# cv-core/MIT-Driverless-CV-TrainingInfra

Hardware: AMD Instinct MI355X
Metric: images/sec training (YOLOv3 416^2 + RektNet 80^2) (higher is better)
Workload: dtype bf16; 1 GPU; CVC-YOLOv3 yolo_baseline 416x416 classes=80, train step (fwd+bwd+Adam), 32 img/GPU; global_batch=32, parallelism=dp1, hipgraph=False, optimizer=FusedAdam

## Files before the change

mit-driverless-cv-traininginfra_amd/csrc/pw_bwd.hip:

```cpp
#include "common.h"
#include "bn_fuse.h"

struct PwbArgs {
  const void* dy; const void* x; const void* wd; void* dx; const void* addsrc; float* ws;
  int ldy, ldx, lddx, ldadd;
  int M, Cin, Cout;
  int slab_px, nslabs, slices;
  BnFuseArgs fuse;
};

namespace {

constexpr int NT = 512, NW = 8;
constexpr int BP = 32;
constexpr int NS = 64;
constexpr int T64 = 2 * 2048 + 128;
constexpr int SPITCH = 136;
typedef __attribute__((address_space(3))) void lds_void_t;
typedef __attribute__((ext_vector_type(4))) short s16x4_t;
typedef __attribute__((ext_vector_type(8))) short s16x8_t;


__device__ __forceinline__ int swz(int row) { return (row >> 1) & 2; }
__device__ __forceinline__ unsigned lds_u32(const unsigned char* p) {
  return (unsigned)(size_t)(const __attribute__((address_space(3))) unsigned char*)p;
}
__device__ __forceinline__ uint2 lds_rd64(unsigned addr) {
  uint2 v;
  asm volatile("ds_read_b64 %0, %1" : "=v"(v) : "v"(addr) : "memory");
  return v;
}
template <int OFF> __device__ __forceinline__ s16x4_t lds_tr16(unsigned addr) {
  s16x4_t v;
  asm volatile("ds_read_b64_tr_b16 %0, %1 offset:%2" : "=v"(v) : "v"(addr), "n"(OFF) : "memory");
  return v;
}

template <int CO4, int S, bool ADD, bool FUSE>
__global__ __launch_bounds__(NT) void pw_bwd_kernel(PwbArgs a) {
  constexpr int KB = 2 * CO4;
  constexpr int NX = 1 + (ADD ? 1 : 0) + (FUSE ? 1 : 0);
  constexpr int WD_BYTES = KB * 4096;
  constexpr int STG = KB * 2048 + NX * T64;
  constexpr int STAGING = WD_BYTES + S * STG;
  constexpr int DUMP = STAGING + BP * SPITCH;
  constexpr int NCHUNK = 2 * KB + 4 * NX;
  constexpr int NPW = (NCHUNK + NW - 1) / NW;
  extern __shared__ __attribute__((aligned(1024))) unsigned char smem[];

  const int xcd = (int)(blockIdx.x & 7), seq = (int)(blockIdx.x >> 3);
  const int slab = xcd + 8 * (seq / a.slices), slice = seq % a.slices;
  if (slab >= a.nslabs) return;
  const int tid = threadIdx.x, lane = tid & 63;
  const int wave = __builtin_amdgcn_readfirstlane(tid >> 6);
  const int px0 = slab * a.slab_px;
  const int px_end = min(a.M, px0 + a.slab_px);
  const int ntiles = (px_end - px0 + BP - 1) / BP;
  const int ci0 = slice * NS;

  const __amdgpu_buffer_rsrc_t rwd = __builtin_amdgcn_make_buffer_rsrc(const_cast<void*>(a.wd), 0, (unsigned)a.Cin * (unsigned)a.Cout * 2u, 0x00020000);

  const int lrow = lane >> 2, lslot = (lane & 3) ^ swz(lrow);
#define PWB_SETUP(I)                                                                                                               \
  const int c##I = wave + NW * I;                                                                                 \
  const int cc##I = c##I - 2 * KB, t##I = cc##I >> 2, b##I = (cc##I >> 1) & 1, g##I = c##I & 1;                                      \
  const bool isdy##I = c##I < 2 * KB, live##I = c##I < NCHUNK;                                                                       \
  const int k##I = isdy##I ? 0 : (t##I == 0 ? 1 : ((ADD && t##I == 1) ? 2 : 3));                      \
  const void* bp##I = k##I == 0 ? a.dy : (k##I == 1 ? a.x : (k##I == 2 ? a.addsrc : a.fuse.y));                                     \
  const unsigned ld##I = (unsigned)(k##I == 0 ? a.ldy : (k##I == 1 ? a.ldx : (k##I == 2 ? a.ldadd : a.fuse.ldy)));                  \
  const unsigned pitch##I = live##I ? ld##I * 2u : 0u;                                                                              \
  const __amdgpu_buffer_rsrc_t rs##I = __builtin_amdgcn_make_buffer_rsrc(const_cast<void*>(live##I ? bp##I : a.dy), 0,              \
                                                                         live##I ? (unsigned)px_end * ld##I * 2u : 0u, 0x00020000); \
  const int ch##I = isdy##I ? (c##I >> 1) * 32 : ci0 + b##I * 32;                                                                   \
  const unsigned voff##I = live##I ? (unsigned)(g##I * 16 + lrow) * pitch##I + (unsigned)(ch##I + lslot * 8) * 2u : 0u;             \
  const unsigned ldso##I = !live##I ? (unsigned)(DUMP - WD_BYTES)                                                                   \
                                    : (isdy##I ? (unsigned)((c##I >> 1) * 2048 + g##I * 1024)                                       \
                                               : (unsigned)(KB * 2048 + t##I * T64 + b##I * (2048 + 128) + g##I * 1024));           \
  const unsigned smul##I = live##I ? (unsigned)STG : 0u;
  PWB_SETUP(0) PWB_SETUP(1) PWB_SETUP(2) PWB_SETUP(3) PWB_SETUP(4) PWB_SETUP(5)
#undef PWB_SETUP
  static_assert(NPW <= 6, "six DMA roles per wave");
#define PWB_ISSUE_ONE(I, PROW_, SLOT_)                                                                                             \
  if constexpr (I < NPW)                                                                                                          \
    __builtin_amdgcn_raw_ptr_buffer_load_lds(rs##I, (lds_void_t*)(smem + WD_BYTES + (unsigned)(SLOT_) * smul##I + ldso##I), 16,      \
                                             (int)voff##I, (int)((PROW_) * pitch##I), 0, 0)
#define PWB_ISSUE_TILE(T_, SLOT_)                                                                                                  \
  do {                                                                                                                           \
    const unsigned prow__ = (unsigned)(px0 + (T_) * BP);                                                                         \
    PWB_ISSUE_ONE(0, prow__, SLOT_); PWB_ISSUE_ONE(1, prow__, SLOT_); PWB_ISSUE_ONE(2, prow__, SLOT_);                           \
    PWB_ISSUE_ONE(3, prow__, SLOT_); PWB_ISSUE_ONE(4, prow__, SLOT_); PWB_ISSUE_ONE(5, prow__, SLOT_);                           \
  } while (0)

#pragma unroll
  for (int i = 0; i < (4 * KB) / NW; ++i) {
    const int c = wave + NW * i, kb = c >> 2, g = c & 3;
    const unsigned vo = (unsigned)(ci0 + g * 16 + lrow) * (unsigned)a.Cout * 2u + (unsigned)(kb * 32 + lslot * 8) * 2u;
    __builtin_amdgcn_raw_ptr_buffer_load_lds(rwd, (lds_void_t*)(smem + kb * 4096 + g * 1024), 16, (int)vo, 0, 0, 0);
  }
  int issued = 0;
  for (; issued < S - 1 && issued < ntiles; ++issued) PWB_ISSUE_TILE(issued, issued);

  const int r16 = lane & 15, q4 = lane >> 4;
  const int offF = r16 * 64 + ((q4 ^ swz(r16)) << 4);
  const int cb = wave & 3, pb = wave >> 2;
  const unsigned char* const pWd = smem + (cb * 16) * 64 + offF;
  const int trow = q4 * 4 + (r16 >> 2);
  const int tsub = (r16 & 1) * 8, tq = (r16 & 3) >> 1;
  const int wc = wave >> 1, wn = wave & 1;
  const int erow = tid >> 4, ecg = tid & 15;
  const int eblk = ecg >> 3, eslot = (ecg & 7) >> 1, esub = (ecg & 1) * 8;
  const int eoff64 = eblk * (2048 + 128) + erow * 64 + ((eslot ^ swz(erow & 15)) << 4) + esub;
  bf16_t* __restrict__ dxp = reinterpret_cast<bf16_t*>(a.dx);
  const unsigned stg_wr = lds_u32(smem) + (unsigned)(STAGING + (pb * 16 + r16) * SPITCH + cb * 32 + q4 * 8);

  float fs[4], fb[4], fm[4], sg[4], sx[4];
  if constexpr (FUSE) {
#pragma unroll
    for (int e = 0; e < 4; ++e) {
      const int n = ci0 + ecg * 4 + e;
      fs[e] = a.fuse.scale[n]; fb[e] = a.fuse.shift[n]; fm[e] = a.fuse.mean[n]; sg[e] = 0.f; sx[e] = 0.f;
    }
  }

  f32x4_t accw[CO4][2];
#pragma unroll
  for (int i = 0; i < CO4; ++i)
#pragma unroll
    for (int j = 0; j < 2; ++j) accw[i][j] = f32x4_t{0.f, 0.f, 0.f, 0.f};

  int slot = 0, islot = issued % S;
  for (int t = 0; t < ntiles; ++t) {
    const int newer = issued - 1 - t;
    if (S > 2 && newer >= S - 2) asm volatile("s_waitcnt vmcnt(%0)" ::"n"((S > 2 ? S - 2 : 0) * NPW) : "memory");
    else asm volatile("s_waitcnt vmcnt(0)" ::: "memory");
    asm volatile("s_waitcnt lgkmcnt(0)" ::: "memory");
    __builtin_amdgcn_s_barrier();
    if (issued < ntiles) {
      PWB_ISSUE_TILE(issued, islot);
      ++issued;
      islot = islot + 1 == S ? 0 : islot + 1;
    }
    const unsigned char* stg = smem + WD_BYTES + slot * STG;

    {
      f32x4_t acc = f32x4_t{0.f, 0.f, 0.f, 0.f};
      const unsigned char* pB = stg + (pb * 16) * 64 + offF;
#pragma unroll
      for (int kb = 0; kb < KB; ++kb) {
        const bf16x8_t fa = *reinterpret_cast<const bf16x8_t*>(pWd + kb * 4096);
        const bf16x8_t fbv = *reinterpret_cast<const bf16x8_t*>(pB + kb * 2048);
        acc = __builtin_amdgcn_mfma_f32_16x16x32_bf16(fa, fbv, acc, 0, 0, 0);
      }
      uint2 pk;
      pk.x = pack_bf16x2(acc[0], acc[1]); pk.y = pack_bf16x2(acc[2], acc[3]);
      asm volatile("ds_write_b64 %0, %1" ::"v"(stg_wr), "v"(pk) : "memory");
    }

    {
      bf16x8_t fx[2], fd[CO4];
      const unsigned xb = lds_u32(stg) + (unsigned)(KB * 2048 + wn * (2048 + 128) + trow * 64 + tsub);
#pragma unroll
      for (int j = 0; j < 2; ++j) {
        const unsigned ad = xb + (unsigned)((((2 * j + tq) ^ swz(trow)) << 4));
        const s16x4_t lo = lds_tr16<0>(ad), hi = lds_tr16<1024>(ad);
        const s16x8_t v = {lo[0], lo[1], lo[2], lo[3], hi[0], hi[1], hi[2], hi[3]};
        fx[j] = __builtin_bit_cast(bf16x8_t, v);
      }
      const unsigned db = lds_u32(stg) + (unsigned)(trow * 64 + tsub);
#pragma unroll
      for (int i = 0; i < CO4; ++i) {
        const int gblk = wc * CO4 + i;
        const unsigned ad = db + (unsigned)((gblk >> 1) * 2048) + (unsigned)((((2 * (gblk & 1) + tq) ^ swz(trow)) << 4));
        const s16x4_t lo = lds_tr16<0>(ad), hi = lds_tr16<1024>(ad);
        const s16x8_t v = {lo[0], lo[1], lo[2], lo[3], hi[0], hi[1], hi[2], hi[3]};
        fd[i] = __builtin_bit_cast(bf16x8_t, v);
      }
      asm volatile("s_waitcnt lgkmcnt(0)" ::: "memory");
#pragma unroll
      for (int j = 0; j < 2; ++j) asm volatile("" : "+v"(fx[j]));
#pragma unroll
      for (int i = 0; i < CO4; ++i) asm volatile("" : "+v"(fd[i]));
#pragma unroll
      for (int i = 0; i < CO4; ++i)
#pragma unroll
        for (int j = 0; j < 2; ++j) accw[i][j] = __builtin_amdgcn_mfma_f32_16x16x32_bf16(fd[i], fx[j], accw[i][j], 0, 0, 0);
    }

    asm volatile("s_waitcnt lgkmcnt(0)" ::: "memory");
    __builtin_amdgcn_s_barrier();
    {
      const int p = px0 + t * BP + erow;
      const unsigned sbase = lds_u32(stg) + (unsigned)(KB * 2048 + eoff64);
      uint2 d = lds_rd64(lds_u32(smem) + (unsigned)(STAGING + erow * SPITCH + ecg * 8)), q = d, yq = d;
      if constexpr (ADD) q = lds_rd64(sbase + T64);
      if constexpr (FUSE) yq = lds_rd64(sbase + (NX - 1) * T64);
      asm volatile("s_waitcnt lgkmcnt(0)" : "+v"(d), "+v"(q), "+v"(yq)::"memory");
      float v[4];
      v[0] = __uint_as_float(d.x << 16); v[1] = __uint_as_float(d.x & 0xffff0000u);
      v[2] = __uint_as_float(d.y << 16); v[3] = __uint_as_float(d.y & 0xffff0000u);
      if constexpr (ADD) {
        v[0] += __uint_as_float(q.x << 16); v[1] += __uint_as_float(q.x & 0xffff0000u);
        v[2] += __uint_as_float(q.y << 16); v[3] += __uint_as_float(q.y & 0xffff0000u);
        d.x = pack_bf16x2(v[0], v[1]); d.y = pack_bf16x2(v[2], v[3]);
      }
      if (p < px_end) *reinterpret_cast<uint2*>(dxp + (size_t)p * a.lddx + ci0 + ecg * 4) = d;
      if constexpr (FUSE) {
        if (p < px_end) {
          float yv[4];
          yv[0] = __uint_as_float(yq.x << 16); yv[1] = __uint_as_float(yq.x & 0xffff0000u);
          yv[2] = __uint_as_float(yq.y << 16); yv[3] = __uint_as_float(yq.y & 0xffff0000u);
          v[0] = __uint_as_float(d.x << 16); v[1] = __uint_as_float(d.x & 0xffff0000u);
          v[2] = __uint_as_float(d.y << 16); v[3] = __uint_as_float(d.y & 0xffff0000u);
#pragma unroll
          for (int e = 0; e < 4; ++e) {
            const float pre = __builtin_fmaf(yv[e], fs[e], fb[e]);
            const float g = (a.fuse.act != 0 && !(pre > 0.f)) ? v[e] * a.fuse.slope : v[e];
            sg[e] += g;
            sx[e] += g * (yv[e] - fm[e]);
          }
        }
      }
    }
    slot = slot + 1 == S ? 0 : slot + 1;
  }

  {
    float* __restrict__ wsp = a.ws + (size_t)slab * a.Cout * a.Cin + ci0 + wn * 32 + r16;
#pragma unroll
    for (int i = 0; i < CO4; ++i)
#pragma unroll
      for (int j = 0; j < 2; ++j)
#pragma unroll
        for (int rr = 0; rr < 4; ++rr) {
          const int co = (wc * CO4 + i) * 16 + q4 * 4 + rr;
          wsp[(size_t)co * a.Cin + j * 16] = accw[i][j][rr];
        }
  }
  if constexpr (FUSE) {
#pragma unroll
    for (int e = 0; e < 4; ++e) {
      sg[e] += __shfl_xor(sg[e], 16, 64); sx[e] += __shfl_xor(sx[e], 16, 64);
      sg[e] += __shfl_xor(sg[e], 32, 64); sx[e] += __shfl_xor(sx[e], 32, 64);
    }
    asm volatile("s_waitcnt vmcnt(0) lgkmcnt(0)" ::: "memory");
    __builtin_amdgcn_s_barrier();
    float* red = reinterpret_cast<float*>(smem + WD_BYTES);
    if (lane < 16) {
#pragma unroll
      for (int e = 0; e < 4; ++e) { red[(wave * 2 + 0) * 64 + lane * 4 + e] = sg[e]; red[(wave * 2 + 1) * 64 + lane * 4 + e] = sx[e]; }
    }
    __syncthreads();
    if (tid < 128) {
      float tot = 0.f;
#pragma unroll
      for (int w = 0; w < NW; ++w) tot += red[w * 128 + tid];
      const int which = tid >> 6, c = tid & 63;
      a.fuse.partial[(size_t)(a.fuse.row_base + slab) * 2 * a.Cin + (size_t)which * a.Cin + ci0 + c] = tot;
    }
  }
}

#undef PWB_ISSUE_TILE
#undef PWB_ISSUE_ONE

template <int CO4, int S, bool ADD, bool FUSE>
int launch_pwb(const PwbArgs& a, hipStream_t st) {
  constexpr int KB = 2 * CO4, NX = 1 + (ADD ? 1 : 0) + (FUSE ? 1 : 0);
  constexpr int LDS = KB * 4096 + S * (KB * 2048 + NX * T64) + BP * SPITCH + 1024;
  static_assert(LDS <= 160 * 1024, "LDS budget");
  auto kern = pw_bwd_kernel<CO4, S, ADD, FUSE>;
  static DynLds dyn_lds;
  if (hipError_t e = mdcv_dyn_lds(dyn_lds, reinterpret_cast<const void*>(kern), LDS); e != hipSuccess) return (int)e;
  const unsigned grid = (unsigned)(8 * cdiv(a.nslabs, 8) * a.slices);
  MDCV_LAUNCH(kern, dim3(grid), dim3(NT), LDS, st, a);
  MDCV_CHECK_LAUNCH();
  return MDCV_OK;
}

template <int CO4, int S>
int launch_pwb2(const PwbArgs& a, hipStream_t st) {
  const bool add = a.addsrc != nullptr, fuse = a.fuse.y != nullptr;
  if (add) return fuse ? launch_pwb<CO4, S, true, true>(a, st) : launch_pwb<CO4, S, true, false>(a, st);
  return fuse ? launch_pwb<CO4, S, false, true>(a, st) : launch_pwb<CO4, S, false, false>(a, st);
}

int device_cus() {
  static int cus[64] = {};
  int dev = 0;
  if (hipGetDevice(&dev) != hipSuccess || dev < 0 || dev >= 64) return 256;
  if (!cus[dev]) {
    int n = 0;
    cus[dev] = (hipDeviceGetAttribute(&n, hipDeviceAttributeMultiprocessorCount, dev) == hipSuccess && n >= 8) ? n : 256;
  }
  return cus[dev];
}

int pwb_lds_bytes(int Cout) {
  const int KB = Cout / 32, S = Cout >= 512 ? 2 : 3;
  return KB * 4096 + S * (KB * 2048 + 3 * T64) + BP * SPITCH + 1024;
}

}

extern "C" {

int mdcv_pw_bwd_slabs(int dtype, long long M, int Cin, int Cout, int ldy, int ldx, int lddx, int ldadd, int ldfy) {
  if (dtype != MDCV_BF16 || M < 1) return 0;
  if (Cout != 64 && Cout != 128 && Cout != 256 && Cout != 512) return 0;
  if (Cin < 64 || (Cin & 63)) return 0;
  if ((ldy & 7) || (ldx & 7) || (lddx & 3) || (ldadd & 7) || (ldfy & 7)) return 0;
  const long long ldmax = (long long)(ldy > ldx ? ldy : ldx) > (ldadd > ldfy ? ldadd : ldfy) ? (ldy > ldx ? ldy : ldx) : (ldadd > ldfy ? ldadd : ldfy);
  if ((M + 64) * ldmax * 2 >= (1LL << 31) || (long long)Cin * Cout * 2 >= (1LL << 31)) return 0;
  const int ncu = device_cus();
  const int per_cu = (160 * 1024) / pwb_lds_bytes(Cout);
  const int slices = Cin / NS;
  const int xcd_slots = (ncu / 8) * (per_cu < 1 ? 1 : per_cu);
  int P = 8 * (xcd_slots / slices > 0 ? xcd_slots / slices : 1);
  long long spx = ((M + P - 1) / P + BP - 1) / BP * BP;
  if (spx < 4 * BP) spx = 4 * BP;
  return (int)((M + spx - 1) / spx);
}

int mdcv_pw_bwd(int dtype, const void* dy, int ldy, const void* x, int ldx, const void* wd_packed, void* dx, int lddx, const void* addsrc,
                int ldadd, float* ws, int slabs, const void* fy, int ldfy, const float* fscale, const float* fshift, const float* fmean, int fact,
                float fslope, float* fpartial, long long M, int Cin, int Cout, void* stream) {
  if (!dy || !x || !wd_packed || !dx || !ws) return MDCV_EARG;
  if (slabs < 1 || slabs != mdcv_pw_bwd_slabs(dtype, M, Cin, Cout, ldy, ldx, lddx, addsrc ? ldadd : 8, fy ? ldfy : 8)) return MDCV_EARG;
  PwbArgs a{};
  a.dy = dy; a.x = x; a.wd = wd_packed; a.dx = dx; a.addsrc = addsrc; a.ws = ws;
  a.ldy = ldy; a.ldx = ldx; a.lddx = lddx; a.ldadd = ldadd;
  a.M = (int)M; a.Cin = Cin; a.Cout = Cout;
  a.nslabs = slabs; a.slices = Cin / NS;
  a.slab_px = (int)(((M + slabs - 1) / slabs + BP - 1) / BP * BP);
  a.fuse = BnFuseArgs{};
  if (fy) {
    if (!fscale || !fshift || !fmean || !fpartial) return MDCV_EARG;
    a.fuse.y = fy; a.fuse.ldy = ldfy; a.fuse.scale = fscale; a.fuse.shift = fshift; a.fuse.mean = fmean; a.fuse.partial = fpartial;
    a.fuse.act = fact; a.fuse.slope = fact == 2 ? 0.f : fslope; a.fuse.row_base = 0;
  }
  hipStream_t st = (hipStream_t)stream;
  switch (Cout) {
    case 64: return launch_pwb2<1, 3>(a, st);
    case 128: return launch_pwb2<2, 3>(a, st);
    case 256: return launch_pwb2<4, 3>(a, st);
    case 512: return launch_pwb2<8, 2>(a, st);
  }
  return MDCV_EARG;
}

}
```

mit-driverless-cv-traininginfra_amd/csrc/tune.h:

```cpp
#pragma once

struct MdcvTune {
  int conv_no_ut = 0;
  int conv_tall_narrow = 256;
  int conv_deep_narrow = 1;
  int conv_deep_small = 8;
  int conv_fuse_narrow = 1;
  int conv_variant = -1;
  int conv_tall_s2 = 1;
  int conv_deep_s2 = 1;
  int conv_s2_allcls = 1;
  int conv_s2_split = 512;
  int conv_s2_split_on = 1;
  int wgrad_slots = 512;
  int wgrad_bna_stages = 2;
  int wgrad_variant = 0;
  int shift_ring = 4;
  int shift_wmax_narrow = 104;
  int shift_wmax_n32 = 0;
  int shift_dil2 = 1;
  int shift_n64 = 2;
  int shift_wmax = 80;
  int shift_loop = 2;
  int shift_2d = 1;
  int shift_big = 0;
  int shift_n64_wide = 1;
  int shift_plan = 0;
  int shift_s2 = 1;
  int pw_bmp = 0;
  int pw_wres = 1;
  int stream_blocks = 0;
  int stream_tiled = 1;
  int stream_light_maxpos = 600000;
  int stream_table = 1;
  int stream_direct = 1;
  int stream_s2 = 1;
  int stream_s2_blocks = 256;
  int stream_s2_depth = 2;
  int stream_s2_lds = 160 * 1024;
  int stream_light_depth = 1;
  int stream_light_blocks = 256;
  int stream_tiled_blocks = 128;
};

extern thread_local const MdcvTune* mdcv_t_tune;
inline const MdcvTune& TUNE() { return *mdcv_t_tune; }

enum { MDCV_TUNE_CONV = 0, MDCV_TUNE_WGRAD = 1, MDCV_TUNE_PW = 2 };

inline void mdcv_tune_shift(MdcvTune& t, int ring) {
  if (ring == 63 || ring == 64) { t.shift_n64_wide = ring - 63; return; }
  if (ring == 29 || ring == 60) { t.shift_s2 = ring == 60; return; }
  if (ring == 27 || ring == 28) { t.shift_2d = ring - 27; return; }
  if (ring >= 200 && ring < 300) { t.shift_big = ring == 201 ? 384 : 0; return; }
  if (ring >= 30 && ring <= 59) { t.shift_loop = ring - 30; return; }
  if (ring == 25 || ring == 26) { t.shift_wmax_n32 = ring == 25 ? 208 : 0; return; }
  if (ring == 23 || ring == 24) { t.shift_wmax_narrow = ring == 23 ? 104 : 0; return; }
  if (ring >= 20 && ring <= 22) { t.shift_dil2 = ring == 20 ? 2 : (ring == 21 ? 0 : 1); return; }
  if (ring >= 17 && ring <= 19) { t.shift_n64 = ring == 17 ? 1 : (ring == 18 ? 0 : 2); return; }
  if (ring >= 14 && ring <= 16) { t.shift_wmax = ring == 14 ? 80 : (ring == 15 ? 62 : 104); return; }
  if (ring >= 7) t.shift_plan = ring - 7;
  else if (ring >= 3 && ring <= 5) t.shift_ring = ring;
}
inline void mdcv_tune_apply_conv(MdcvTune& t, int v) {
  if (v == 0) return;
  if (v <= -3 && v >= -299) { mdcv_tune_shift(t, -v); return; }
  if (v == 93 || v == 92) { t.conv_fuse_narrow = v == 93; return; }
  if (v >= 60 && v < 92) { t.conv_deep_small = v - 60; return; }
  if (v >= 30 && v < 60) { t.conv_deep_narrow = v - 30; return; }
  if (v == 20 || v == 21) { t.conv_deep_s2 = v - 20; return; }
  if (v == 16 || v == 17) { t.conv_s2_allcls = v - 16; return; }
  if (v == 14 || v == 15) { t.conv_s2_split_on = v - 14; return; }
  if (v >= 4000 && v < 6000) { t.conv_s2_split = v - 4000; return; }
  if (v == 18 || v == 19) { t.conv_tall_s2 = v - 18; return; }
  if (v >= 2000 && v < 3000) { t.conv_tall_narrow = v - 2000; return; }
  if (v >= 100) { t.conv_no_ut = 1; v -= 100; }
  if (v >= 1 && v <= 12) t.conv_variant = v - 1;
}
inline void mdcv_tune_apply_wgrad(MdcvTune& t, int v) {
  if (v == 0) return;
  if (v >= 20000 && v < 30000) { t.wgrad_slots = v - 20000; return; }
  if (v >= 35000 && v < 36000) { t.stream_s2_blocks = v - 35000; return; }
  if (v >= 30000 && v < 40000) {
    const int b = v - 30000;
    if (b >= 4001 && b <= 4002) { t.stream_light_depth = b - 4000; return; }
    if (b >= 4012 && b <= 4014) { t.wgrad_bna_stages = b - 4010; return; }
    if (b == 4020 || b == 4021) { t.stream_table = b - 4020; return; }
    if (b == 4050 || b == 4051) { t.stream_direct = b - 4050; return; }
    if (b == 4060 || b == 4061) { t.stream_s2 = b - 4060; return; }
    if (b >= 4071 && b <= 4073) { t.stream_s2_depth = b - 4070; return; }
    if (b >= 4100 && b <= 4260) { t.stream_s2_lds = (b - 4100) * 1024; return; }
    if (b == 2) t.stream_light_maxpos = 600000;
    else if (b == 3) t.stream_light_maxpos = 1 << 30;
    else if (b == 5) t.stream_light_maxpos = 0;
    else if (b >= 3000 && b < 4000) t.stream_light_blocks = b - 3000;
    else t.stream_tiled_blocks = b > 0 ? b : 128;
    return;
  }
  if (v >= 1000) { const int d = (v - 1000) / 100; t.stream_tiled = !(d & 8); t.stream_blocks = ((v - 1000) % 100) * 64; return; }
  t.wgrad_variant = v;
}
inline void mdcv_tune_apply_pw(MdcvTune& t, int v) {
  if (v == 1000 || v == 1001) { t.pw_wres = v - 1000; return; }
  if (v == 64 || v == 32 || v == 16) t.pw_bmp = v;
}

struct TuneScope {
  MdcvTune t;
  const MdcvTune* prev;
  int dtype;
  TuneScope(int dtype_arg, int family) : prev(mdcv_t_tune), dtype(dtype_arg & 0xff) {
    const int code = dtype_arg >> 8;
    if (code != 0) {
      if (family == MDCV_TUNE_CONV) mdcv_tune_apply_conv(t, code);
      else if (family == MDCV_TUNE_WGRAD) mdcv_tune_apply_wgrad(t, code);
      else mdcv_tune_apply_pw(t, code);
      mdcv_t_tune = &t;
    }
  }
  explicit TuneScope(const MdcvTune& forced) : t(forced), prev(mdcv_t_tune), dtype(0) { mdcv_t_tune = &t; }
  ~TuneScope() { mdcv_t_tune = prev; }
  TuneScope(const TuneScope&) = delete;
  TuneScope& operator=(const TuneScope&) = delete;
};
#define MDCV_TUNE_ENTRY(dtype_var, family) const TuneScope tune_scope__((dtype_var), (family)); (dtype_var) = tune_scope__.dtype
```

mit-driverless-cv-traininginfra_amd/engine.py:

```python
import os

import torch

from . import _lib
from ._lib import F32, BF16, ACT_NONE, ACT_LEAKY, ACT_RELU, tuned


_POISON = os.environ.get("MDCV_POISON", "0") == "1"
_REDZONE = int(os.environ.get("MDCV_REDZONE", "0"))
_RZ_BYTE = 0xA5


def _alloc(n, dtype, device, zero, plan):
    if not _REDZONE:
        t = (torch.zeros if zero else torch.empty)(n, dtype=dtype, device=device)
        if not zero and _POISON and t.is_floating_point():
            t.fill_(float("nan"))
        return t
    es = torch.empty(0, dtype=dtype).element_size()
    raw = torch.full((n * es + _REDZONE,), _RZ_BYTE, dtype=torch.uint8, device=device)
    t = raw[:n * es].view(dtype)
    if zero:
        t.zero_()
    plan.__dict__.setdefault("redzones", []).append((raw, n * es))
# ... 261 lines not shown
        self.call(lst, self.L.bn_act_fwd, self.dtype, a.ptr, a.ldc, None, None, None, 0, None, None, b.ptr if b is not None else None,
                  b.ldc if b is not None else 0, out.ptr, out.ldc, out.M, out.C, ACT_NONE, 0.0)

    def _alloc_like(self, a):
        return self.new_act(a.B, a.H, a.W, a.C)

    def emit_input(self, B, C, H, W):
        a = self.new_act(B, H, W, C)
        node = TNode(a, needs_grad=False, name="input")
        holder = {"src": None}
        L, dt = self.L, self.dtype

        def convert(stream):
            x = holder["src"]
            return L.nchw_to_nhwc(dt, x.data_ptr(), a.ptr, B, C, H, W, a.ldc, a.C, stream)
        convert.__name__ = "nchw_to_nhwc"
        self.fwd.append((convert, ()))
        return node, holder

    def emit_pack(self, cs, need_dgrad):
        if need_dgrad and cs.wd is None:
            cs.wd = _alloc(cs.cin_pad * cs.kh * cs.kw * cs.cout_pad, self.tdtype, self.device, True, self)
        self.pack_list.append(cs)
        self.layer_marks.append(len(self.fwd))

    def stats_rows(self, cs, x, y):
        return int(self.L.conv2d_stats_rows_geom(self.cdt, x.B, y.H, y.W, cs.cin_pad, cs.cout_pad, cs.kh, cs.kw, cs.stride, cs.pad,
                                                 cs.dil, x.ldc))

    def emit_conv_fwd(self, cs, x, y, stats_partial=None):
        assert x.C == cs.cin_pad and y.C == cs.cout_pad, (x.C, cs.cin_pad, y.C, cs.cout_pad)
        self.call(self.fwd, self.L.conv2d, self.cdt, 0, x.ptr, x.ldc, cs.wf.data_ptr(), y.ptr, y.ldc,
                  cs.bias_pad.data_ptr() if cs.bias_pad is not None else None, None, 0,
                  stats_partial.data_ptr() if stats_partial is not None else None,
                  x.B, x.H, x.W, cs.cin_pad, y.H, y.W, cs.cout_pad, cs.kh, cs.kw, cs.stride, cs.pad, cs.dil)

    def emit_conv_bwd(self, cs, xnode, y_shape_act, dy, x_wgrad=None):
        L, dt = self.L, self.dtype
        x = xnode.act
        if x_wgrad is None and self._emit_pw_bwd1(cs, xnode, dy):
            return
        xw = x_wgrad if x_wgrad is not None else x
        cin_w = xw.C if x_wgrad is not None else cs.cin_pad
        if self.wgrad_after_dgrad and cs.kh == 3 and cs.stride == 1:
            self._emit_dgrad(cs, xnode, dy)
            self._emit_wgrad_single(cs, xw, dy, cin_w)
        else:
            self._emit_wgrad_single(cs, xw, dy, cin_w)
            self._emit_dgrad(cs, xnode, dy)

    wgrad_after_dgrad = False

    pw_bwd1 = True

    def _emit_pw_bwd1(self, cs, xnode, dy):
        L, dt = self.L, self.dtype
        x = xnode.act
        if not self.pw_bwd1 or dt != BF16 or not xnode.needs_grad or cs.wd is None:
            return False
        if (cs.kh, cs.kw, cs.stride, cs.pad) != (1, 1, 1, 0) or x.C != cs.cin_pad or dy.C != cs.cout_pad:
            return False
        slabs = int(L.pw_bwd_slabs(dt, x.M, cs.cin_pad, cs.cout_pad, dy.ldc, x.ldc, 8, 8, 8))
        if slabs < 1:
            return False
        out, add = self.grad_target(xnode)
        assert slabs == int(L.pw_bwd_slabs(dt, x.M, cs.cin_pad, cs.cout_pad, dy.ldc, x.ldc, out.ldc, add.ldc if add is not None else 8, 8))
        gw = self.param_grad(cs.weight)
        ws = self.f32(slabs * cs.cout_pad * cs.cin_pad, zero=False)
        args = [dt, dy.ptr, dy.ldc, x.ptr, x.ldc, cs.wd.data_ptr(), out.ptr, out.ldc, add.ptr if add is not None else None,
                add.ldc if add is not None else 0, ws.data_ptr(), slabs, None, 0, None, None, None, 0, 0.0, None, x.M, cs.cin_pad, cs.cout_pad]
        self.dgrad_entries[out.ptr] = dict(
            idx=len(self.bwd), out=out, used=False, pwb=args,
            geom=(x.B, dy.H, dy.W, cs.cout_pad, x.H, x.W, cs.cin_pad, cs.kh, cs.kw, cs.stride, cs.pad, cs.dil), head=(dy.ptr, dy.ldc))
        self.call(self.bwd, L.pw_bwd, *args)

        def wreduce(stream, ws=ws, gw=gw, slabs=slabs, cs=cs):
            return L.wgrad_reduce(ws.data_ptr(), slabs, gw.data_ptr(), 0, cs.cout_pad, cs.cout, cs.cin_pad, cs.cin, 1, stream)
        wreduce.__name__ = "conv2d_wgrad"
        wreduce.info = (x.B, x.H, x.W, cs.cin_pad, dy.H, dy.W, cs.cout_pad, 0, 1, slabs)
        self.bwd.append((wreduce, ()))
        self.pw_bwd1_count = getattr(self, "pw_bwd1_count", 0) + 1
        return True

    def _emit_wgrad_single(self, cs, xw, dy, cin_w):
        L, dt = self.L, self.dtype
        gw = self.param_grad(cs.weight)
        splits = int(L.conv2d_wgrad_splits_geom(self.wdt, xw.B, xw.H, xw.W, cin_w, dy.H, dy.W, cs.cout_pad, cs.kh, cs.kw, cs.stride, cs.pad,
                                                cs.dil, dy.ldc, xw.ldc))
        self.ws_floats = max(self.ws_floats, splits * cs.cout_pad * cs.kh * cs.kw * cin_w)
        plan = self

        def wgrad(stream, cs=cs, x=xw, dy=dy, gw=gw, splits=splits, cin_w=cin_w):
            return L.conv2d_wgrad(plan.wdt, dy.ptr, dy.ldc, x.ptr, x.ldc, plan.wgrad_ws(stream).data_ptr(), splits, gw.data_ptr(), 0,
                                  x.B, x.H, x.W, cin_w, cs.cin, dy.H, dy.W, cs.cout_pad, cs.cout, cs.kh, cs.kw,
                                  cs.stride, cs.pad, cs.dil, stream)
        wgrad.__name__ = "conv2d_wgrad"
        wgrad.info = (xw.B, xw.H, xw.W, cin_w, dy.H, dy.W, cs.cout_pad, cs.kh, cs.stride, splits)
        self.bwd.append((wgrad, ()))

    def _emit_dgrad(self, cs, xnode, dy):
        L, dt = self.L, self.dtype
        x = xnode.act
        if xnode.needs_grad:
            out, add = self.grad_target(xnode)
            self.dgrad_entries[out.ptr] = dict(
                idx=len(self.bwd), out=out, used=False,
                geom=(x.B, dy.H, dy.W, cs.cout_pad, x.H, x.W, cs.cin_pad, cs.kh, cs.kw, cs.stride, cs.pad, cs.dil),
                head=(dy.ptr, dy.ldc, cs.wd.data_ptr(), out.ptr, out.ldc, add.ptr if add is not None else None,
                      add.ldc if add is not None else 0))
            self.call(self.bwd, L.conv2d, self.cdt, 1, dy.ptr, dy.ldc, cs.wd.data_ptr(), out.ptr, out.ldc, None,
                      add.ptr if add is not None else None, add.ldc if add is not None else 0, None,
                      x.B, dy.H, dy.W, cs.cout_pad, x.H, x.W, cs.cin_pad, cs.kh, cs.kw, cs.stride, cs.pad, cs.dil)

    def emit_bias_grad(self, cs, dy, zero_only=False):
        gb = self.param_grad(cs.bias)
        if zero_only:
            gb.zero_()
            return
        tmp = self.f32(cs.cout_pad)
        pws = self.f32(int(self.L.colsum_ws_floats(self.dtype, dy.M, cs.cout_pad)), zero=False)
        self.call(self.bwd, self.L.colsum_f32, self.dtype, dy.ptr, dy.ldc, dy.M, cs.cout_pad, pws.data_ptr(), tmp.data_ptr())

# ... 415 lines not shown
```

Measured before the change: 2494 images/sec.

## Add 128-channel-wide Cin slices to fused pointwise backward kernel

```diff
diff --git a/mit-driverless-cv-traininginfra_amd/csrc/pw_bwd.hip b/mit-driverless-cv-traininginfra_amd/csrc/pw_bwd.hip
--- a/mit-driverless-cv-traininginfra_amd/csrc/pw_bwd.hip
+++ b/mit-driverless-cv-traininginfra_amd/csrc/pw_bwd.hip
@@ -36,16 +36,22 @@
   return v;
 }
 
-template <int CO4, int S, bool ADD, bool FUSE>
+constexpr int pwb_lds(int KB, int S, int H, int NX) { return H * KB * 4096 + S * (KB * 2048 + NX * H * T64) + H * BP * SPITCH + 1024; }
+
+template <int CO4, int S, int NS2, bool ADD, bool FUSE>
 __global__ __launch_bounds__(NT) void pw_bwd_kernel(PwbArgs a) {
+  static_assert(NS2 == 64 || NS2 == 128, "one or two 64-channel halves");
+  constexpr int H = NS2 / NS;
   constexpr int KB = 2 * CO4;
   constexpr int NX = 1 + (ADD ? 1 : 0) + (FUSE ? 1 : 0);
-  constexpr int WD_BYTES = KB * 4096;
-  constexpr int STG = KB * 2048 + NX * T64;
+  constexpr int WD_HALF = KB * 4096;
+  constexpr int WD_BYTES = H * WD_HALF;
+  constexpr int STG = KB * 2048 + NX * H * T64;
   constexpr int STAGING = WD_BYTES + S * STG;
-  constexpr int DUMP = STAGING + BP * SPITCH;
-  constexpr int NCHUNK = 2 * KB + 4 * NX;
+  constexpr int DUMP = STAGING + H * BP * SPITCH;
+  constexpr int NCHUNK = 2 * KB + 4 * NX * H;
   constexpr int NPW = (NCHUNK + NW - 1) / NW;
+  static_assert(DUMP + 1024 == pwb_lds(KB, S, H, NX), "launch_pwb sizes the same layout");
   extern __shared__ __attribute__((aligned(1024))) unsigned char smem[];
 
   const int xcd = (int)(blockIdx.x & 7), seq = (int)(blockIdx.x >> 3);
@@ -56,14 +62,15 @@
   const int px0 = slab * a.slab_px;
   const int px_end = min(a.M, px0 + a.slab_px);
   const int ntiles = (px_end - px0 + BP - 1) / BP;
-  const int ci0 = slice * NS;
+  const int ci0 = slice * NS2;
 
   const __amdgpu_buffer_rsrc_t rwd = __builtin_amdgcn_make_buffer_rsrc(const_cast<void*>(a.wd), 0, (unsigned)a.Cin * (unsigned)a.Cout * 2u, 0x00020000);
 
   const int lrow = lane >> 2, lslot = (lane & 3) ^ swz(lrow);
 #define PWB_SETUP(I)                                                                                                               \
   const int c##I = wave + NW * I;                                                                                 \
-  const int cc##I = c##I - 2 * KB, t##I = cc##I >> 2, b##I = (cc##I >> 1) & 1, g##I = c##I & 1;                                      \
+  const int cc##I = c##I - 2 * KB, im##I = cc##I >> 2, b##I = (cc##I >> 1) & 1, g##I = c##I & 1;                                     \
+  const int t##I = im##I / H, hh##I = im##I % H;                                                    \
   const bool isdy##I = c##I < 2 * KB, live##I = c##I < NCHUNK;                                                                       \
   const int k##I = isdy##I ? 0 : (t##I == 0 ? 1 : ((ADD && t##I == 1) ? 2 : 3));                      \
   const void* bp##I = k##I == 0 ? a.dy : (k##I == 1 ? a.x : (k##I == 2 ? a.addsrc : a.fuse.y));                                     \
@@ -71,11 +78,11 @@
   const unsigned pitch##I = live##I ? ld##I * 2u : 0u;                                                                              \
   const __amdgpu_buffer_rsrc_t rs##I = __builtin_amdgcn_make_buffer_rsrc(const_cast<void*>(live##I ? bp##I : a.dy), 0,              \
                                                                          live##I ? (unsigned)px_end * ld##I * 2u : 0u, 0x00020000); \
-  const int ch##I = isdy##I ? (c##I >> 1) * 32 : ci0 + b##I * 32;                                                                   \
+  const int ch##I = isdy##I ? (c##I >> 1) * 32 : ci0 + hh##I * NS + b##I * 32;                                                      \
   const unsigned voff##I = live##I ? (unsigned)(g##I * 16 + lrow) * pitch##I + (unsigned)(ch##I + lslot * 8) * 2u : 0u;             \
   const unsigned ldso##I = !live##I ? (unsigned)(DUMP - WD_BYTES)                                                                   \
                                     : (isdy##I ? (unsigned)((c##I >> 1) * 2048 + g##I * 1024)                                       \
-                                               : (unsigned)(KB * 2048 + t##I * T64 + b##I * (2048 + 128) + g##I * 1024));           \
+                                               : (unsigned)(KB * 2048 + im##I * T64 + b##I * (2048 + 128) + g##I * 1024));          \
   const unsigned smul##I = live##I ? (unsigned)STG : 0u;
   PWB_SETUP(0) PWB_SETUP(1) PWB_SETUP(2) PWB_SETUP(3) PWB_SETUP(4) PWB_SETUP(5)
 #undef PWB_SETUP
@@ -92,10 +99,10 @@
   } while (0)
 
 #pragma unroll
-  for (int i = 0; i < (4 * KB) / NW; ++i) {
-    const int c = wave + NW * i, kb = c >> 2, g = c & 3;
-    const unsigned vo = (unsigned)(ci0 + g * 16 + lrow) * (unsigned)a.Cout * 2u + (unsigned)(kb * 32 + lslot * 8) * 2u;
-    __builtin_amdgcn_raw_ptr_buffer_load_lds(rwd, (lds_void_t*)(smem + kb * 4096 + g * 1024), 16, (int)vo, 0, 0, 0);
+  for (int i = 0; i < (H * 4 * KB) / NW; ++i) {
+    const int c = wave + NW * i, hw = c / (4 * KB), kb = (c % (4 * KB)) >> 2, g = c & 3;
+    const unsigned vo = (unsigned)(ci0 + hw * NS + g * 16 + lrow) * (unsigned)a.Cout * 2u + (unsigned)(kb * 32 + lslot * 8) * 2u;
+    __builtin_amdgcn_raw_ptr_buffer_load_lds(rwd, (lds_void_t*)(smem + hw * WD_HALF + kb * 4096 + g * 1024), 16, (int)vo, 0, 0, 0);
   }
   int issued = 0;
   for (; issued < S - 1 && issued < ntiles; ++issued) PWB_ISSUE_TILE(issued, issued);
@@ -112,21 +119,26 @@
   const int eoff64 = eblk * (2048 + 128) + erow * 64 + ((eslot ^ swz(erow & 15)) << 4) + esub;
   bf16_t* __restrict__ dxp = reinterpret_cast<bf16_t*>(a.dx);
   const unsigned stg_wr = lds_u32(smem) + (unsigned)(STAGING + (pb * 16 + r16) * SPITCH + cb * 32 + q4 * 8);
-
-  float fs[4], fb[4], fm[4], sg[4], sx[4];
+  const unsigned stg_rd = lds_u32(smem) + (unsigned)(STAGING + erow * SPITCH + ecg * 8);
+
+  float fs[H][4], fb[H][4], fm[H][4], sg[H][4], sx[H][4];
   if constexpr (FUSE) {
 #pragma unroll
-    for (int e = 0; e < 4; ++e) {
-      const int n = ci0 + ecg * 4 + e;
-      fs[e] = a.fuse.scale[n]; fb[e] = a.fuse.shift[n]; fm[e] = a.fuse.mean[n]; sg[e] = 0.f; sx[e] = 0.f;
-    }
-  }
-
-  f32x4_t accw[CO4][2];
-#pragma unroll
-  for (int i = 0; i < CO4; ++i)
-#pragma unroll
-    for (int j = 0; j < 2; ++j) accw[i][j] = f32x4_t{0.f, 0.f, 0.f, 0.f};
+    for (int h = 0; h < H; ++h)
+#pragma unroll
+      for (int e = 0; e < 4; ++e) {
+        const int n = ci0 + h * NS + ecg * 4 + e;
+        fs[h][e] = a.fuse.scale[n]; fb[h][e] = a.fuse.shift[n]; fm[h][e] = a.fuse.mean[n]; sg[h][e] = 0.f; sx[h][e] = 0.f;
+      }
+  }
+
+  f32x4_t accw[H][CO4][2];
+#pragma unroll
+  for (int h = 0; h < H; ++h)
+#pragma unroll
+    for (int i = 0; i < CO4; ++i)
+#pragma unroll
+      for (int j = 0; j < 2; ++j) accw[h][i][j] = f32x4_t{0.f, 0.f, 0.f, 0.f};
 
   int slot = 0, islot = issued % S;
   for (int t = 0; t < ntiles; ++t) {
@@ -143,28 +155,39 @@
     const unsigned char* stg = smem + WD_BYTES + slot * STG;
 
     {
-      f32x4_t acc = f32x4_t{0.f, 0.f, 0.f, 0.f};
+      f32x4_t acc[H];
+#pragma unroll
+      for (int h = 0; h < H; ++h) acc[h] = f32x4_t{0.f, 0.f, 0.f, 0.f};
       const unsigned char* pB = stg + (pb * 16) * 64 + offF;
 #pragma unroll
       for (int kb = 0; kb < KB; ++kb) {
-        const bf16x8_t fa = *reinterpret_cast<const bf16x8_t*>(pWd + kb * 4096);
         const bf16x8_t fbv = *reinterpret_cast<const bf16x8_t*>(pB + kb * 2048);
-        acc = __builtin_amdgcn_mfma_f32_16x16x32_bf16(fa, fbv, acc, 0, 0, 0);
-      }
-      uint2 pk;
-      pk.x = pack_bf16x2(acc[0], acc[1]); pk.y = pack_bf16x2(acc[2], acc[3]);
-      asm volatile("ds_write_b64 %0, %1" ::"v"(stg_wr), "v"(pk) : "memory");
+#pragma unroll
+        for (int h = 0; h < H; ++h) {
+          const bf16x8_t fa = *reinterpret_cast<const bf16x8_t*>(pWd + h * WD_HALF + kb * 4096);
+          acc[h] = __builtin_amdgcn_mfma_f32_16x16x32_bf16(fa, fbv, acc[h], 0, 0, 0);
+        }
+      }
+#pragma unroll
+      for (int h = 0; h < H; ++h) {
+        uint2 pk;
+        pk.x = pack_bf16x2(acc[h][0], acc[h][1]); pk.y = pack_bf16x2(acc[h][2], acc[h][3]);
+        asm volatile("ds_write_b64 %0, %1" ::"v"(stg_wr + (unsigned)(h * BP * SPITCH)), "v"(pk) : "memory");
+      }
     }
 
     {
-      bf16x8_t fx[2], fd[CO4];
-      const unsigned xb = lds_u32(stg) + (unsigned)(KB * 2048 + wn * (2048 + 128) + trow * 64 + tsub);
-#pragma unroll
-      for (int j = 0; j < 2; ++j) {
-        const unsigned ad = xb + (unsigned)((((2 * j + tq) ^ swz(trow)) << 4));
-        const s16x4_t lo = lds_tr16<0>(ad), hi = lds_tr16<1024>(ad);
-        const s16x8_t v = {lo[0], lo[1], lo[2], lo[3], hi[0], hi[1], hi[2], hi[3]};
-        fx[j] = __builtin_bit_cast(bf16x8_t, v);
+      bf16x8_t fx[H][2], fd[CO4];
+#pragma unroll
+      for (int h = 0; h < H; ++h) {
+        const unsigned xb = lds_u32(stg) + (unsigned)(KB * 2048 + h * T64 + wn * (2048 + 128) + trow * 64 + tsub);
+#pragma unroll
+        for (int j = 0; j < 2; ++j) {
+          const unsigned ad = xb + (unsigned)((((2 * j + tq) ^ swz(trow)) << 4));
+          const s16x4_t lo = lds_tr16<0>(ad), hi = lds_tr16<1024>(ad);
+          const s16x8_t v = {lo[0], lo[1], lo[2], lo[3], hi[0], hi[1], hi[2], hi[3]};
+          fx[h][j] = __builtin_bit_cast(bf16x8_t, v);
+        }
       }
       const unsigned db = lds_u32(stg) + (unsigned)(trow * 64 + tsub);
 #pragma unroll
@@ -177,13 +200,17 @@
       }
       asm volatile("s_waitcnt lgkmcnt(0)" ::: "memory");
 #pragma unroll
-      for (int j = 0; j < 2; ++j) asm volatile("" : "+v"(fx[j]));
+      for (int h = 0; h < H; ++h)
+#pragma unroll
+        for (int j = 0; j < 2; ++j) asm volatile("" : "+v"(fx[h][j]));
 #pragma unroll
       for (int i = 0; i < CO4; ++i) asm volatile("" : "+v"(fd[i]));
 #pragma unroll
-      for (int i = 0; i < CO4; ++i)
-#pragma unroll
-        for (int j = 0; j < 2; ++j) accw[i][j] = __builtin_amdgcn_mfma_f32_16x16x32_bf16(fd[i], fx[j], accw[i][j], 0, 0, 0);
+      for (int h = 0; h < H; ++h)
+#pragma unroll
+        for (int i = 0; i < CO4; ++i)
+#pragma unroll
+          for (int j = 0; j < 2; ++j) accw[h][i][j] = __builtin_amdgcn_mfma_f32_16x16x32_bf16(fd[i], fx[h][j], accw[h][i][j], 0, 0, 0);
     }
 
     asm volatile("s_waitcnt lgkmcnt(0)" ::: "memory");
@@ -191,32 +218,41 @@
     {
       const int p = px0 + t * BP + erow;
       const unsigned sbase = lds_u32(stg) + (unsigned)(KB * 2048 + eoff64);
-      uint2 d = lds_rd64(lds_u32(smem) + (unsigned)(STAGING + erow * SPITCH + ecg * 8)), q = d, yq = d;
-      if constexpr (ADD) q = lds_rd64(sbase + T64);
-      if constexpr (FUSE) yq = lds_rd64(sbase + (NX - 1) * T64);
-      asm volatile("s_waitcnt lgkmcnt(0)" : "+v"(d), "+v"(q), "+v"(yq)::"memory");
-      float v[4];
-      v[0] = __uint_as_float(d.x << 16); v[1] = __uint_as_float(d.x & 0xffff0000u);
-      v[2] = __uint_as_float(d.y << 16); v[3] = __uint_as_float(d.y & 0xffff0000u);
-      if constexpr (ADD) {
-        v[0] += __uint_as_float(q.x << 16); v[1] += __uint_as_float(q.x & 0xffff0000u);
-        v[2] += __uint_as_float(q.y << 16); v[3] += __uint_as_float(q.y & 0xffff0000u);
-        d.x = pack_bf16x2(v[0], v[1]); d.y = pack_bf16x2(v[2], v[3]);
-      }
-      if (p < px_end) *reinterpret_cast<uint2*>(dxp + (size_t)p * a.lddx + ci0 + ecg * 4) = d;
-      if constexpr (FUSE) {
-        if (p < px_end) {
-          float yv[4];
-          yv[0] = __uint_as_float(yq.x << 16); yv[1] = __uint_as_float(yq.x & 0xffff0000u);
-          yv[2] = __uint_as_float(yq.y << 16); yv[3] = __uint_as_float(yq.y & 0xffff0000u);
-          v[0] = __uint_as_float(d.x << 16); v[1] = __uint_as_float(d.x & 0xffff0000u);
-          v[2] = __uint_as_float(d.y << 16); v[3] = __uint_as_float(d.y & 0xffff0000u);
-#pragma unroll
-          for (int e = 0; e < 4; ++e) {
-            const float pre = __builtin_fmaf(yv[e], fs[e], fb[e]);
-            const float g = (a.fuse.act != 0 && !(pre > 0.f)) ? v[e] * a.fuse.slope : v[e];
-            sg[e] += g;
-            sx[e] += g * (yv[e] - fm[e]);
+      uint2 d[H], q[H], yq[H];
+#pragma unroll
+      for (int h = 0; h < H; ++h) {
+        d[h] = lds_rd64(stg_rd + (unsigned)(h * BP * SPITCH)); q[h] = d[h]; yq[h] = d[h];
+        if constexpr (ADD) q[h] = lds_rd64(sbase + (unsigned)((H + h) * T64));
+        if constexpr (FUSE) yq[h] = lds_rd64(sbase + (unsigned)(((NX - 1) * H + h) * T64));
+      }
+      asm volatile("s_waitcnt lgkmcnt(0)" ::: "memory");
+#pragma unroll
+      for (int h = 0; h < H; ++h) asm volatile("" : "+v"(d[h]), "+v"(q[h]), "+v"(yq[h]));
+#pragma unroll
+      for (int h = 0; h < H; ++h) {
+        float v[4];
+        v[0] = __uint_as_float(d[h].x << 16); v[1] = __uint_as_float(d[h].x & 0xffff0000u);
+        v[2] = __uint_as_float(d[h].y << 16); v[3] = __uint_as_float(d[h].y & 0xffff0000u);
+        if constexpr (ADD) {
+          v[0] += __uint_as_float(q[h].x << 16); v[1] += __uint_as_float(q[h].x & 0xffff0000u);
+          v[2] += __uint_as_float(q[h].y << 16); v[3] += __uint_as_float(q[h].y & 0xffff0000u);
+          d[h].x = pack_bf16x2(v[0], v[1]); d[h].y = pack_bf16x2(v[2], v[3]);
+        }
+        if (p < px_end) *reinterpret_cast<uint2*>(dxp + (size_t)p * a.lddx + ci0 + h * NS + ecg * 4) = d[h];
+        if constexpr (FUSE) {
+          if (p < px_end) {
+            float yv[4];
+            yv[0] = __uint_as_float(yq[h].x << 16); yv[1] = __uint_as_float(yq[h].x & 0xffff0000u);
+            yv[2] = __uint_as_float(yq[h].y << 16); yv[3] = __uint_as_float(yq[h].y & 0xffff0000u);
+            v[0] = __uint_as_float(d[h].x << 16); v[1] = __uint_as_float(d[h].x & 0xffff0000u);
+            v[2] = __uint_as_float(d[h].y << 16); v[3] = __uint_as_float(d[h].y & 0xffff0000u);
+#pragma unroll
+            for (int e = 0; e < 4; ++e) {
+              const float pre = __builtin_fmaf(yv[e], fs[h][e], fb[h][e]);
+              const float g = (a.fuse.act != 0 && !(pre > 0.f)) ? v[e] * a.fuse.slope : v[e];
+              sg[h][e] += g;
+              sx[h][e] += g * (yv[e] - fm[h][e]);
+            }
           }
         }
       }
@@ -225,36 +261,46 @@
   }
 
   {
-    float* __restrict__ wsp = a.ws + (size_t)slab * a.Cout * a.Cin + ci0 + wn * 32 + r16;
-#pragma unroll
-    for (int i = 0; i < CO4; ++i)
-#pragma unroll
-      for (int j = 0; j < 2; ++j)
-#pragma unroll
-        for (int rr = 0; rr < 4; ++rr) {
-          const int co = (wc * CO4 + i) * 16 + q4 * 4 + rr;
-          wsp[(size_t)co * a.Cin + j * 16] = accw[i][j][rr];
-        }
+#pragma unroll
+    for (int h = 0; h < H; ++h) {
+      float* __restrict__ wsp = a.ws + (size_t)slab * a.Cout * a.Cin + ci0 + h * NS + wn * 32 + r16;
+#pragma unroll
+      for (int i = 0; i < CO4; ++i)
+#pragma unroll
+        for (int j = 0; j < 2; ++j)
+#pragma unroll
+          for (int rr = 0; rr < 4; ++rr) {
+            const int co = (wc * CO4 + i) * 16 + q4 * 4 + rr;
+            wsp[(size_t)co * a.Cin + j * 16] = accw[h][i][j][rr];
+          }
+    }
   }
   if constexpr (FUSE) {
 #pragma unroll
-    for (int e = 0; e < 4; ++e) {
-      sg[e] += __shfl_xor(sg[e], 16, 64); sx[e] += __shfl_xor(sx[e], 16, 64);
-      sg[e] += __shfl_xor(sg[e], 32, 64); sx[e] += __shfl_xor(sx[e], 32, 64);
-    }
+    for (int h = 0; h < H; ++h)
+#pragma unroll
+      for (int e = 0; e < 4; ++e) {
+        sg[h][e] += __shfl_xor(sg[h][e], 16, 64); sx[h][e] += __shfl_xor(sx[h][e], 16, 64);
+        sg[h][e] += __shfl_xor(sg[h][e], 32, 64); sx[h][e] += __shfl_xor(sx[h][e], 32, 64);
+      }
     asm volatile("s_waitcnt vmcnt(0) lgkmcnt(0)" ::: "memory");
     __builtin_amdgcn_s_barrier();
     float* red = reinterpret_cast<float*>(smem + WD_BYTES);
+    static_assert(NW * 2 * NS2 * 4 <= S * STG, "the wave sums fit the ring");
     if (lane < 16) {
 #pragma unroll
-      for (int e = 0; e < 4; ++e) { red[(wave * 2 + 0) * 64 + lane * 4 + e] = sg[e]; red[(wave * 2 + 1) * 64 + lane * 4 + e] = sx[e]; }
+      for (int h = 0; h < H; ++h)
+#pragma unroll
+        for (int e = 0; e < 4; ++e) {
+          red[(wave * 2 + 0) * NS2 + h * NS + lane * 4 + e] = sg[h][e]; red[(wave * 2 + 1) * NS2 + h * NS + lane * 4 + e] = sx[h][e];
+        }
     }
     __syncthreads();
-    if (tid < 128) {
+    if (tid < 2 * NS2) {
       float tot = 0.f;
 #pragma unroll
-      for (int w = 0; w < NW; ++w) tot += red[w * 128 + tid];
-      const int which = tid >> 6, c = tid & 63;
+      for (int w = 0; w < NW; ++w) tot += red[w * 2 * NS2 + tid];
+      const int which = tid / NS2, c = tid % NS2;
       a.fuse.partial[(size_t)(a.fuse.row_base + slab) * 2 * a.Cin + (size_t)which * a.Cin + ci0 + c] = tot;
     }
   }
@@ -263,12 +309,12 @@
 #undef PWB_ISSUE_TILE
 #undef PWB_ISSUE_ONE
 
-template <int CO4, int S, bool ADD, bool FUSE>
+template <int CO4, int S, int NS2, bool ADD, bool FUSE>
 int launch_pwb(const PwbArgs& a, hipStream_t st) {
   constexpr int KB = 2 * CO4, NX = 1 + (ADD ? 1 : 0) + (FUSE ? 1 : 0);
-  constexpr int LDS = KB * 4096 + S * (KB * 2048 + NX * T64) + BP * SPITCH + 1024;
+  constexpr int LDS = pwb_lds(KB, S, NS2 / NS, NX);
   static_assert(LDS <= 160 * 1024, "LDS budget");
-  auto kern = pw_bwd_kernel<CO4, S, ADD, FUSE>;
+  auto kern = pw_bwd_kernel<CO4, S, NS2, ADD, FUSE>;
   static DynLds dyn_lds;
   if (hipError_t e = mdcv_dyn_lds(dyn_lds, reinterpret_cast<const void*>(kern), LDS); e != hipSuccess) return (int)e;
   const unsigned grid = (unsigned)(8 * cdiv(a.nslabs, 8) * a.slices);
@@ -277,11 +323,11 @@
   return MDCV_OK;
 }
 
-template <int CO4, int S>
+template <int CO4, int S, int NS2>
 int launch_pwb2(const PwbArgs& a, hipStream_t st) {
   const bool add = a.addsrc != nullptr, fuse = a.fuse.y != nullptr;
-  if (add) return fuse ? launch_pwb<CO4, S, true, true>(a, st) : launch_pwb<CO4, S, true, false>(a, st);
-  return fuse ? launch_pwb<CO4, S, false, true>(a, st) : launch_pwb<CO4, S, false, false>(a, st);
+  if (add) return fuse ? launch_pwb<CO4, S, NS2, true, true>(a, st) : launch_pwb<CO4, S, NS2, true, false>(a, st);
+  return fuse ? launch_pwb<CO4, S, NS2, false, true>(a, st) : launch_pwb<CO4, S, NS2, false, false>(a, st);
 }
 
 int device_cus() {
@@ -295,25 +341,35 @@
   return cus[dev];
 }
 
-int pwb_lds_bytes(int Cout) {
-  const int KB = Cout / 32, S = Cout >= 512 ? 2 : 3;
-  return KB * 4096 + S * (KB * 2048 + 3 * T64) + BP * SPITCH + 1024;
-}
-
-}
-
-extern "C" {
-
-int mdcv_pw_bwd_slabs(int dtype, long long M, int Cin, int Cout, int ldy, int ldx, int lddx, int ldadd, int ldfy) {
-  if (dtype != MDCV_BF16 || M < 1) return 0;
+constexpr int pwb_stages(int Cout, bool wide) { return (Cout >= 512 || (wide && Cout >= 256)) ? 2 : 3; }
+static_assert(pwb_lds(8, pwb_stages(256, true), 2, 3) == 158720 && pwb_lds(8, 3, 2, 3) > 160 * 1024, "128-wide slices at Cout = 256: two stages fit, three do not");
+
+int pwb_lds_bytes(int Cout, bool wide) { return pwb_lds(Cout / 32, pwb_stages(Cout, wide), wide ? 2 : 1, 3); }
+
+bool pwb_wide_pays(long long M, int Cin, int Cout) {
+  if (M < 16384) return false;
+  if (M < 65536) return Cout == 256;
+  return true;
+}
+
+int pwb_slice_width(long long M, int Cin, int Cout) {
+  const int mode = TUNE().pwb_wide;
+  const bool fits = (Cin % 128) == 0 && Cout <= 256;
+  if (!fits || mode == 0) return NS;
+  return (mode == 2 || pwb_wide_pays(M, Cin, Cout)) ? 2 * NS : NS;
+}
+
+int pwb_slabs(long long M, int Cin, int Cout, int ldy, int ldx, int lddx, int ldadd, int ldfy) {
+  if (M < 1) return 0;
   if (Cout != 64 && Cout != 128 && Cout != 256 && Cout != 512) return 0;
   if (Cin < 64 || (Cin & 63)) return 0;
   if ((ldy & 7) || (ldx & 7) || (lddx & 3) || (ldadd & 7) || (ldfy & 7)) return 0;
   const long long ldmax = (long long)(ldy > ldx ? ldy : ldx) > (ldadd > ldfy ? ldadd : ldfy) ? (ldy > ldx ? ldy : ldx) : (ldadd > ldfy ? ldadd : ldfy);
   if ((M + 64) * ldmax * 2 >= (1LL << 31) || (long long)Cin * Cout * 2 >= (1LL << 31)) return 0;
   const int ncu = device_cus();
-  const int per_cu = (160 * 1024) / pwb_lds_bytes(Cout);
-  const int slices = Cin / NS;
+  const int ns2 = pwb_slice_width(M, Cin, Cout);
+  const int per_cu = (160 * 1024) / pwb_lds_bytes(Cout, ns2 > NS);
+  const int slices = Cin / ns2;
   const int xcd_slots = (ncu / 8) * (per_cu < 1 ? 1 : per_cu);
   int P = 8 * (xcd_slots / slices > 0 ? xcd_slots / slices : 1);
   long long spx = ((M + P - 1) / P + BP - 1) / BP * BP;
@@ -321,16 +377,28 @@
   return (int)((M + spx - 1) / spx);
 }
 
+}
+
+extern "C" {
+
+int mdcv_pw_bwd_slabs(int dtype, long long M, int Cin, int Cout, int ldy, int ldx, int lddx, int ldadd, int ldfy) {
+  MDCV_TUNE_ENTRY(dtype, MDCV_TUNE_PW);
+  if (dtype != MDCV_BF16) return 0;
+  return pwb_slabs(M, Cin, Cout, ldy, ldx, lddx, ldadd, ldfy);
+}
+
 int mdcv_pw_bwd(int dtype, const void* dy, int ldy, const void* x, int ldx, const void* wd_packed, void* dx, int lddx, const void* addsrc,
                 int ldadd, float* ws, int slabs, const void* fy, int ldfy, const float* fscale, const float* fshift, const float* fmean, int fact,
                 float fslope, float* fpartial, long long M, int Cin, int Cout, void* stream) {
-  if (!dy || !x || !wd_packed || !dx || !ws) return MDCV_EARG;
-  if (slabs < 1 || slabs != mdcv_pw_bwd_slabs(dtype, M, Cin, Cout, ldy, ldx, lddx, addsrc ? ldadd : 8, fy ? ldfy : 8)) return MDCV_EARG;
+  MDCV_TUNE_ENTRY(dtype, MDCV_TUNE_PW);
+  if (!dy || !x || !wd_packed || !dx || !ws || dtype != MDCV_BF16) return MDCV_EARG;
+  if (slabs < 1 || slabs != pwb_slabs(M, Cin, Cout, ldy, ldx, lddx, addsrc ? ldadd : 8, fy ? ldfy : 8)) return MDCV_EARG;
+  const int ns2 = pwb_slice_width(M, Cin, Cout);
   PwbArgs a{};
   a.dy = dy; a.x = x; a.wd = wd_packed; a.dx = dx; a.addsrc = addsrc; a.ws = ws;
   a.ldy = ldy; a.ldx = ldx; a.lddx = lddx; a.ldadd = ldadd;
   a.M = (int)M; a.Cin = Cin; a.Cout = Cout;
-  a.nslabs = slabs; a.slices = Cin / NS;
+  a.nslabs = slabs; a.slices = Cin / ns2;
   a.slab_px = (int)(((M + slabs - 1) / slabs + BP - 1) / BP * BP);
   a.fuse = BnFuseArgs{};
   if (fy) {
@@ -339,11 +407,19 @@
     a.fuse.act = fact; a.fuse.slope = fact == 2 ? 0.f : fslope; a.fuse.row_base = 0;
   }
   hipStream_t st = (hipStream_t)stream;
+  if (ns2 == 2 * NS) {
+    switch (Cout) {
+      case 64: return launch_pwb2<1, pwb_stages(64, true), 128>(a, st);
+      case 128: return launch_pwb2<2, pwb_stages(128, true), 128>(a, st);
+      case 256: return launch_pwb2<4, pwb_stages(256, true), 128>(a, st);
+    }
+    return MDCV_EARG;
+  }
   switch (Cout) {
-    case 64: return launch_pwb2<1, 3>(a, st);
-    case 128: return launch_pwb2<2, 3>(a, st);
-    case 256: return launch_pwb2<4, 3>(a, st);
-    case 512: return launch_pwb2<8, 2>(a, st);
+    case 64: return launch_pwb2<1, pwb_stages(64, false), 64>(a, st);
+    case 128: return launch_pwb2<2, pwb_stages(128, false), 64>(a, st);
+    case 256: return launch_pwb2<4, pwb_stages(256, false), 64>(a, st);
+    case 512: return launch_pwb2<8, pwb_stages(512, false), 64>(a, st);
   }
   return MDCV_EARG;
 }
diff --git a/mit-driverless-cv-traininginfra_amd/csrc/tune.h b/mit-driverless-cv-traininginfra_amd/csrc/tune.h
--- a/mit-driverless-cv-traininginfra_amd/csrc/tune.h
+++ b/mit-driverless-cv-traininginfra_amd/csrc/tune.h
@@ -29,6 +29,7 @@
   int shift_s2 = 1;
   int pw_bmp = 0;
   int pw_wres = 1;
+  int pwb_wide = 1;
   int stream_blocks = 0;
   int stream_tiled = 1;
   int stream_light_maxpos = 600000;
@@ -102,6 +103,7 @@
 }
 inline void mdcv_tune_apply_pw(MdcvTune& t, int v) {
   if (v == 1000 || v == 1001) { t.pw_wres = v - 1000; return; }
+  if (v >= 2000 && v <= 2002) { t.pwb_wide = v - 2000; return; }
   if (v == 64 || v == 32 || v == 16) t.pw_bmp = v;
 }
 
diff --git a/mit-driverless-cv-traininginfra_amd/engine.py b/mit-driverless-cv-traininginfra_amd/engine.py
--- a/mit-driverless-cv-traininginfra_amd/engine.py
+++ b/mit-driverless-cv-traininginfra_amd/engine.py
@@ -337,6 +337,7 @@
     wgrad_after_dgrad = False
 
     pw_bwd1 = True
+    pw_bwd_code = 0
 
     def _emit_pw_bwd1(self, cs, xnode, dy):
         L, dt = self.L, self.dtype
@@ -345,14 +346,15 @@
             return False
         if (cs.kh, cs.kw, cs.stride, cs.pad) != (1, 1, 1, 0) or x.C != cs.cin_pad or dy.C != cs.cout_pad:
             return False
-        slabs = int(L.pw_bwd_slabs(dt, x.M, cs.cin_pad, cs.cout_pad, dy.ldc, x.ldc, 8, 8, 8))
+        pdt = tuned(dt, self.pw_bwd_code)
+        slabs = int(L.pw_bwd_slabs(pdt, x.M, cs.cin_pad, cs.cout_pad, dy.ldc, x.ldc, 8, 8, 8))
         if slabs < 1:
             return False
         out, add = self.grad_target(xnode)
-        assert slabs == int(L.pw_bwd_slabs(dt, x.M, cs.cin_pad, cs.cout_pad, dy.ldc, x.ldc, out.ldc, add.ldc if add is not None else 8, 8))
+        assert slabs == int(L.pw_bwd_slabs(pdt, x.M, cs.cin_pad, cs.cout_pad, dy.ldc, x.ldc, out.ldc, add.ldc if add is not None else 8, 8))
         gw = self.param_grad(cs.weight)
         ws = self.f32(slabs * cs.cout_pad * cs.cin_pad, zero=False)
-        args = [dt, dy.ptr, dy.ldc, x.ptr, x.ldc, cs.wd.data_ptr(), out.ptr, out.ldc, add.ptr if add is not None else None,
+        args = [pdt, dy.ptr, dy.ldc, x.ptr, x.ldc, cs.wd.data_ptr(), out.ptr, out.ldc, add.ptr if add is not None else None,
                 add.ldc if add is not None else 0, ws.data_ptr(), slabs, None, 0, None, None, None, 0, 0.0, None, x.M, cs.cin_pad, cs.cout_pad]
         self.dgrad_entries[out.ptr] = dict(
             idx=len(self.bwd), out=out, used=False, pwb=args,
```

Result: no change. 2509 images/sec (median of 6 runs) (+0.6%).
